# Dave-he/unet-watermark

Hardware: AMD Instinct MI355X
Metric: train_images_per_sec (higher is better)
Workload: dtype f32 storage and accumulation; the convolution products of the encoder and decoder layers (3x3, 7x7 stem, stride-2 and 1x1 layers: forward, data gradients, and the weight gradients of the stride-1 3x3 layers and the stem) as fp16x3 splits - every fp32 operand = two fp16 halves (22 mantissa bits), a*b; 1 GPU; Unet-resnet34 512x512 bs16/GPU train step: fwd + Dice + bwd + Adam (BASELINE.json configs[1]); global_batch=16, parallelism=dp1, grad_allreduce=none

## Files before the change

unet-watermark_amd/_lib.py:

```python
from __future__ import annotations

import ctypes as C
import os
import subprocess
import sys
from pathlib import Path

os.environ.setdefault("GPU_MAX_HW_QUEUES", "8")

_PKG_DIR = Path(__file__).resolve().parent
_CSRC = _PKG_DIR / "csrc"
LIB_PATH = _PKG_DIR / "libuwm.so"
SOURCES = ["uwm_route.hip", "conv_igemm.hip", "conv_patch.hip", "conv_patch16.hip", "conv_wino.hip", "conv_wino8.hip", "conv_wino_x3.hip", "conv_f16x3.hip", "conv_f16x3v2.hip", "conv_stem_f16x3.hip", "conv_up2.hip", "conv_up2_f16.hip", "conv_c16_f16.hip", "conv_gemm.hip", "conv_head.hip", "mbconv.hip", "wgrad_igemm.hip", "wgrad_patch.hip", "wgrad_wino.hip", "wgrad_f16x3.hip", "wgrad_c16.hip", "wgrad_gemm.hip", "wgrad_stem.hip", "elementwise.hip", "loss.hip", "loss_ext.hip", "mask_post.hip", "mask_enhance.hip", "resize_u8.hip", "pair_mask_u8.hip", "synth_u8.hip", "synth_text_u8.hip", "extract_u8.hip", "text_enhance.hip", "filter_u8.hip", "augment_u8.hip", "augment_ext_u8.hip", "jpeg_u8.hip", "uwm_model.hip"]
HIP_ARCH = "gfx950"
EXTRA_FLAGS = {name: ["-Xclang", "-target-feature", "-Xclang", "-packed-fp32-ops"]
               for name in ("conv_f16x3.hip", "conv_f16x3v2.hip", "wgrad_f16x3.hip", "conv_stem_f16x3.hip")}
EXTRA_FLAGS["synth_u8.hip"] = ["-ffp-contract=off"]
EXTRA_FLAGS["synth_text_u8.hip"] = ["-ffp-contract=off"]
EXTRA_FLAGS["extract_u8.hip"] = ["-ffp-contract=off"]
EXTRA_FLAGS["text_enhance.hip"] = ["-ffp-contract=off"]


class uwm_unet_desc(C.Structure):
    _fields_ = [("encoder", C.c_int), ("in_channels", C.c_int), ("classes", C.c_int),
                ("decoder_channels", C.c_int * 5), ("bn_eps", C.c_float), ("bn_momentum", C.c_float), ("arch", C.c_int)]


class uwm_tensor_info(C.Structure):
    _fields_ = [("name", C.c_char * 96), ("kind", C.c_int), ("arena", C.c_int), ("ndim", C.c_int),
                ("offset", C.c_longlong), ("shape", C.c_longlong * 4), ("stride", C.c_longlong * 4)]


class uwm_src(C.Structure):
    _fields_ = [("ptr", C.c_void_p), ("scale", C.c_void_p), ("shift", C.c_void_p),
                ("C", C.c_int), ("H", C.c_int), ("W", C.c_int), ("up", C.c_int), ("relu", C.c_int)]

# ... 252 lines not shown
```

unet-watermark_amd/csrc/elementwise.hip:

```cpp
#include "uwm_kernels.h"
#include <vector>
#include <mutex>
#include <cstdlib>

namespace uwm {

typedef float f4 __attribute__((ext_vector_type(4)));
static constexpr int kMaxBlocks = 256 * 8;

static inline unsigned nblocks(size_t work, int per_block) {
  size_t b = (work + per_block - 1) / per_block;
  if (b > (size_t)kMaxBlocks) b = kMaxBlocks;
  if (b < 1) b = 1;
  return (unsigned)b;
}

__global__ void nchw_to_nhwc4_kernel(const float* __restrict__ x, float* __restrict__ y, int C, size_t HW,
                                     size_t total, int CP) {
  for (size_t i = blockIdx.x * (size_t)blockDim.x + threadIdx.x; i < total; i += (size_t)gridDim.x * blockDim.x) {
    const size_t n = i / HW, p = i - n * HW;
    const float* xp = x + n * C * HW + p;
    float* yp = y + i * CP;
    for (int c0 = 0; c0 < CP; c0 += 4) {
      f4 v;
// ... 800 lines not shown
}
const char* prof_class_name(int cls) {
  static const char* names[kProfClasses] = {
      "conv_igemm_kernel<128,128,2,2>", "conv_igemm_kernel<128,64,2,2>", "conv_igemm_kernel<128,32,4,1>",
      "conv_igemm_kernel<128,16,4,1>",  "conv_igemm_kernel<64,64,2,2>",  "conv_igemm_kernel<64,128,1,4>",
      "wgrad_igemm_kernel<64,128,2,2>", "wgrad_igemm_kernel<128,128,2,2>", "wgrad_igemm_kernel<16,256,1,4>",
      "wgrad_igemm_kernel<32,256,1,4>", "conv_patch_kernel<128,2,2>", "conv_patch_kernel<64,2,2>",
      "conv_patch_kernel<32,4,1>",      "conv_patch_kernel<16,4,1>",      "wgrad_patch_kernel<16>",
      "wgrad_patch_kernel<32>",         "wgrad_patch_kernel<64>",         "conv_patch16_kernel<16>",
      "conv_patch16_kernel<32>",        "conv_wino_kernel<64>",           "conv_wino_kernel<32>",
      "conv_wino_kernel<16>",           "wgrad_wino2_kernel<64>",         "wgrad_wino2_kernel<32>",
      "wgrad_wino_kernel<16>",          "conv_wino8_kernel",              "wgrad_igemm_kernel<128,32,2,2>",
      "wgrad_igemm_kernel<128,64,2,2>",  "wgrad_igemm_kernel<32,64,2,2>",  "wgrad_igemm_kernel<32,128,1,4>",
      "conv_head_kernel",               "conv_wino_x3_kernel",            "wgrad_c16_kernel",
      "wgrad_head_kernel",              "conv_up2_kernel",                "conv_up2_dgrad_kernel",
      "wgrad_up2_kernel",               "conv_gemm_kernel<128>",          "conv_gemm_kernel<64>",
      "wgrad_gemm_kernel<128>",         "wgrad_gemm_kernel<64>",          "wgrad_stem_kernel",
      "conv_f16x3_kernel",              "wgrad_f16x3_kernel",             "conv_stem_f16x3_kernel",
      "conv_up2_f16x3_kernel",          "conv_up2_dgrad_f16x3_kernel",    "wgrad_up2_f16x3_kernel",
      "conv_c16_f16x3_kernel",          "wgrad_c16_f16x3_kernel",         "wgrad_stem_f16x3_kernel",
      "conv_gemm_f16x3_kernel<128>",    "conv_gemm_f16x3_kernel<64>",
      "conv_igemm_f16x3_kernel<128,128,2,2>", "conv_igemm_f16x3_kernel<128,64,2,2>", "conv_igemm_f16x3_kernel<128,32,4,1>",
      "conv_igemm_f16x3_kernel<128,16,4,1>",  "conv_igemm_f16x3_kernel<64,64,2,2>",  "conv_igemm_f16x3_kernel<64,128,1,4>",
      "?", "wgrad_igemm_f16x3_kernel<128,128,2,2>", "wgrad_igemm_f16x3_kernel<128,64,2,2>", "wgrad_igemm_f16x3_kernel<64,128,2,2>", "?"};
  return (cls >= 0 && cls < kProfClasses) ? names[cls] : "?";
}

}
```

unet-watermark_amd/csrc/uwm_abi.inc:

```
extern "C" {

const char* uwm_last_error(void) { return g_err; }
int uwm_version(void) { return 1; }

int uwm_create(const uwm_unet_desc* desc, uwm_handle* out) {
  if (!desc || !out) return fail("uwm_create: null argument");
  uwm_model* m = new uwm_model();
  m->desc = *desc;
  if (m->desc.bn_eps <= 0.f) m->desc.bn_eps = 1e-5f;
  if (m->desc.bn_momentum <= 0.f) m->desc.bn_momentum = 0.1f;
  if (build_model(m)) { delete m; return 1; }
  const char* e = getenv("UWM_SIDE_STREAM");
  m->use_side = e ? atoi(e) : 1;
  if (const char* pe = getenv("UWM_PRECISION")) {
    static const char* names[7] = {"f32", "bf16x3", "bf16x3_all", "f16x3", "f16x3_all", "f16x1", "f16x3_bwd2"};
    int found = -1;
    for (int i = 0; i < 7; ++i) if (!strcmp(pe, names[i]) || (pe[0] == '0' + i && !pe[1])) found = i;
    if (found < 0) { delete m; return fail("uwm_create: UWM_PRECISION=%s is not a precision mode (f32 | bf16x3 | bf16x3_all | f16x3 | f16x3_all | f16x1 | f16x3_bwd2 or 0..6)", pe); }
    m->prec = found; m->plan.prec = found; m->prec_from_env = found != UWM_PREC_F32;
  }
  if (const char* pf = getenv("UWM_F16X3_MIN_WGS")) m->f3_min_wgs = atoi(pf) > 0 ? atoi(pf) : 0;
  m->wino_mode = winograd_mode();
  m->plan.wino_mode = m->wino_mode;
  *out = m; return 0;
// ... 1091 lines not shown
    if (rc != 0) return fail("uwm_allreduce_grads: ncclAllReduce failed on bucket %d (ncclResult_t %d)", k, rc);
  }
  return 0;
}
float* uwm_grad_arena(uwm_handle h) { return h ? h->grads : nullptr; }
static Src to_src(const uwm_src* s) { return mk_src(s->ptr, s->C, s->H, s->W, s->scale, s->shift, s->relu, s->up); }

static int g_op_ig16 = 0;
static int op_ig_bank(const float* w, int rows, int Kpad, int slot, hipStream_t st, const float** bank) {
  static float* buf[2] = {nullptr, nullptr}; static size_t cap[2] = {0, 0};
  const size_t n = (size_t)rows * Kpad;
  if (n > cap[slot]) {
    if (buf[slot]) HIPCHK(hipFree(buf[slot]));
    buf[slot] = nullptr; cap[slot] = 0;
    HIPCHK(hipMalloc((void**)&buf[slot], n * sizeof(float)));
    cap[slot] = n;
  }
  WinoJobs jobs; memset(&jobs, 0, sizeof(jobs)); jobs.n = 1;
  jobs.j[0].w = w; jobs.j[0].ut = buf[slot]; jobs.j[0].rows = rows; jobs.j[0].Kpad = Kpad; jobs.j[0].mode = 3; jobs.j[0].src_rows = rows;
  LCHK(launch_f16x3_weights_multi(jobs, st));
  *bank = buf[slot];
  return 0;
}
int uwm_op_set_igemm_f16x3(int on) { g_op_ig16 = on == 2 ? 2 : (on != 0); return 0; }
int uwm_op_conv(const uwm_src* s0, const uwm_src* s1, const float* w, int wrows, int Kpad, int kh, int kw, int stride,
                int pad, int N, int Cout, const float* bias, float* y, double* stats, int cfg, uwm_stream stream) {
  if (!s0 || !w || !y) return fail("uwm_op_conv: null argument");
  ConvArgs a; memset(&a, 0, sizeof(a));
  a.s0 = to_src(s0); a.C0 = a.s0.C;
  if (s1) { a.s1 = to_src(s1); a.Ctot = a.C0 + a.s1.C; } else { a.s1 = a.s0; a.Ctot = a.C0; }
  a.Hl = a.s0.H << a.s0.up; a.Wl = a.s0.W << a.s0.up;
  a.w = w; a.wrows = wrows; a.Kpad = Kpad; a.ntaps = kh * kw; a.kw = kw;
  a.N = N; a.Ho = (a.Hl + 2 * pad - kh) / stride + 1; a.Wo = (a.Wl + 2 * pad - kw) / stride + 1;
  a.Cout = Cout; a.M = N * a.Ho * a.Wo;
  a.smul = stride; a.rmul = 1; a.off = -pad; a.sdiv = 1;
  a.out = y; a.bias = bias;
  if (stats) { a.ssum = stats; a.ssq = stats + Cout; }
  a.dv_ctot = make_fastdiv(a.Ctot); a.dv_kw = make_fastdiv(a.kw);
  a.ig16 = g_op_ig16 != 0;
  if (g_op_ig16 == 1 && !(Kpad & 31) && cfg < 6 && conv_route(a, cfg).k == kConvIgemm && op_ig_bank(w, wrows, Kpad, 0, (hipStream_t)stream, &a.wbank)) return 1;
  if (cfg == 610) {
    static float* sbuf = nullptr;
    if (!sbuf) HIPCHK(hipMalloc((void**)&sbuf, stem_f16x3_bank_floats() * sizeof(float)));
    if (kh != 7 || kw != 7 || a.Ctot != 4 || wrows != 64) return fail("uwm_op_conv: cfg 610 is the 7x7 stem (4 stored input channels, 64 outputs)");
    LCHK(launch_stem_f16x3_weights(w, Kpad, a.Ctot, sbuf, (hipStream_t)stream));
    a.wu = sbuf;
    LCHK(launch_conv_stem_f16x3(a, (hipStream_t)stream));
// ... 10 lines not shown
  } else if (cfg >= 300 && cfg < 500) return fail("uwm_op_conv: cfg 300 (Winograd) needs 3x3 s1 p1, channels %% 8 == 0, Ho >= 8, Wo >= 16");
  LCHK(launch_conv(a, (hipStream_t)stream, cfg));
  return 0;
}
int uwm_op_dgrad(const float* dy, int N, int Ho, int Wo, int Cout, const float* wd, int Cin, int KpadD, int kh, int kw,
                 int stride, int pad, int H, int W, const float* addend, const float* mask, const float* mscale,
                 const float* mshift, float* dx, uwm_stream stream) {
  if (!dy || !wd || !dx) return fail("uwm_op_dgrad: null argument");
  ConvArgs a; memset(&a, 0, sizeof(a));
  a.s0 = mk_src(dy, Cout, Ho, Wo); a.s1 = a.s0; a.C0 = Cout; a.Ctot = Cout;
  a.w = wd; a.wrows = Cin; a.Kpad = KpadD; a.ntaps = kh * kw; a.kw = kw;
  a.N = N; a.Ho = H; a.Wo = W; a.Cout = Cin; a.M = N * H * W;
  a.Hl = Ho; a.Wl = Wo; a.smul = 1; a.rmul = -1; a.off = pad; a.sdiv = stride;
  a.out = dx; a.addend = addend; a.mask = mask; a.mscale = mscale; a.mshift = mshift;
  a.dv_ctot = make_fastdiv(a.Ctot); a.dv_kw = make_fastdiv(a.kw);
  if (g_op_ig16) {
    static float* xm = nullptr;
    if (!xm) HIPCHK(hipMalloc((void**)&xm, 32 * sizeof(float)));
    LCHK(launch_absmax32(dy, (size_t)N * Ho * Wo * Cout, xm, (hipStream_t)stream));
    a.ig16 = 1; a.xmax = xm;
  }
  if (winograd_mode() != 0 && op_wino_shape(a, kh, kw, stride, pad) && op_wino_prepare(a, 1, (hipStream_t)stream)) return 1;
  if (g_op_ig16 == 1 && !(KpadD & 31)) {
    const ConvKernel k = conv_route(a, -1).k;
    if ((k == kConvIgemm || k == kConvS2Dgrad) && op_ig_bank(wd, Cin, KpadD, 0, (hipStream_t)stream, &a.wbank)) return 1;
  }
  LCHK(launch_conv(a, (hipStream_t)stream));
  return 0;
}
int uwm_op_dgrad_upsplit(const float* dy, int N, int H, int W, int Cout, const float* wd, int C0, int C1, int KpadD,
                         float* gprev, const float* pmask, const float* pscale, const float* pshift, float* gskip,
                         uwm_stream stream) {
  if (!dy || !wd || !gprev || (C1 > 0 && !gskip)) return fail("uwm_op_dgrad_upsplit: null argument");
  ConvArgs a; memset(&a, 0, sizeof(a));
  a.s0 = mk_src(dy, Cout, H, W); a.s1 = a.s0; a.C0 = Cout; a.Ctot = Cout;
  a.w = wd; a.wrows = C0 + C1; a.Kpad = KpadD; a.ntaps = 9; a.kw = 3;
  a.N = N; a.Ho = H; a.Wo = W; a.Cout = C0 + C1; a.M = N * H * W;
  a.Hl = H; a.Wl = W; a.smul = 1; a.rmul = -1; a.off = 1; a.sdiv = 1;
  a.out = gskip; a.out_up = gprev; a.up_c0 = C0; a.up_mask = pmask; a.up_mscale = pscale; a.up_mshift = pshift;
  a.dv_ctot = make_fastdiv(a.Ctot); a.dv_kw = make_fastdiv(a.kw);
  if (!op_wino_shape(a, 3, 3, 1, 1) || (H & 1) || (W & 1)) return fail("uwm_op_dgrad_upsplit: needs even H >= 8, W >= 16, channels %% 8 == 0");
  if (g_op_ig16) {
    static float* xm = nullptr;
    if (!xm) HIPCHK(hipMalloc((void**)&xm, 32 * sizeof(float)));
    LCHK(launch_absmax32(dy, (size_t)N * H * W * Cout, xm, (hipStream_t)stream));
    a.ig16 = 1; a.xmax = xm;
  }
  if (op_wino_prepare(a, 1, (hipStream_t)stream)) return 1;
  LCHK(launch_conv(a, (hipStream_t)stream));
  return 0;
// ... 130 lines not shown
```

unet-watermark_amd/csrc/uwm_kernels.h:

```cpp
#pragma once
#include <hip/hip_runtime.h>
#include <hip/hip_ext.h>
#include <stdint.h>
#include <stddef.h>
#include <atomic>

struct uwm_loss_spec;

namespace uwm {

struct Src {
  const float* ptr;
  const float* scale;
  const float* shift;
  int C, H, W;
  int up;
  int relu;
};

struct FastDiv {
  unsigned mg, d;
};
static inline FastDiv make_fastdiv(unsigned d) {
  FastDiv f; f.d = d; f.mg = (d <= 1) ? 0u : (unsigned)((0x100000000ull / d) + 1ull); return f;
// ... 29 lines not shown
  const float* mscale; const float* mshift;
  double* ssum; double* ssq;
  int srep, sstride;
  const float* bnb_mean; const float* bnb_rstd;
  const float* bnb_y;
  FastDiv dv_ctot, dv_kw;
  double flops;
  double bytes;
  float* out_up; int up_c0; const float* up_mask; const float* up_mscale; const float* up_mshift;
  int up_accum;
  int pc_ntaps[4]; unsigned pc_taps[4];
  int live_ch;
  const float* wu;
  int wu_ncb;
  int wino;
  int prec;
  int wu_rinv_off;
  const float* xmax;
  int route_n;
  int ig16;
  int nprod;
  const float* wbank;
  int wu_layout;
};

template <class A> static inline int route_N(const A& a) { return a.route_n > 0 ? a.route_n : a.N; }
template <class A> static inline long route_M(const A& a) { return a.N > 0 ? (long)a.M / a.N * route_N(a) : (long)a.M; }

#if defined(__HIPCC__)
typedef unsigned uwm_u2 __attribute__((ext_vector_type(2)));
__device__ __forceinline__ void uwm_split4(float x0, float x1, float x2, float x3, uwm_u2& hi, uwm_u2& lo) {
  typedef _Float16 h2_ __attribute__((ext_vector_type(2)));
  const h2_ a = {(_Float16)x0, (_Float16)x1}, b = {(_Float16)x2, (_Float16)x3};
  hi.x = __builtin_bit_cast(unsigned, a); hi.y = __builtin_bit_cast(unsigned, b);
  unsigned l0, l1;
  asm("v_fma_mixlo_f16 %0, %1, -1.0, %2 op_sel_hi:[1,0,0]\n\t"
      "v_fma_mixhi_f16 %0, %1, -1.0, %3 op_sel:[1,0,0] op_sel_hi:[1,0,0]"
      : "=&v"(l0) : "v"(hi.x), "v"(x0), "v"(x1));
  asm("v_fma_mixlo_f16 %0, %1, -1.0, %2 op_sel_hi:[1,0,0]\n\t"
      "v_fma_mixhi_f16 %0, %1, -1.0, %3 op_sel:[1,0,0] op_sel_hi:[1,0,0]"
      : "=&v"(l1) : "v"(hi.y), "v"(x2), "v"(x3));
  lo.x = l0; lo.y = l1;
}
constexpr float kIgWScale = 4096.f;
__device__ __forceinline__ void ig_bank_unit(const float* __restrict__ src, float* __restrict__ dst, size_t i, int Kpad) {
  typedef float f4_ __attribute__((ext_vector_type(4)));
// ... 40 lines not shown
  int nprod;
};

enum { kProfClasses = 64 };
void prof_enable(bool on);
bool prof_on();
void prof_pair(int cls, double flops, double bytes, hipEvent_t* e0, hipEvent_t* e1);
void route_note(const char* kernel);
const char* route_last();
#define UWM_LAUNCH(cls, flops, bytes, kernel, grid, block, lds, st, ...)                                     \
  do {                                                                                                       \
    route_note(#kernel);                                                                                     \
    if (prof_on()) {                                                                                         \
      hipEvent_t e0_, e1_; prof_pair((cls), (flops), (bytes), &e0_, &e1_);                                   \
      hipExtLaunchKernelGGL(kernel, grid, block, lds, st, e0_, e1_, 0, __VA_ARGS__);                         \
    } else {                                                                                                 \
      hipLaunchKernelGGL(kernel, grid, block, lds, st, __VA_ARGS__);                                         \
    }                                                                                                        \
  } while (0)
int  prof_collect(double* out );
const char* prof_class_name(int cls);

enum ConvKernel { kConvInvalid = 0, kConvUp2, kConvUp2F16, kConvUp2Dgrad, kConvUp2DgradF16, kConvC16F16, kConvC32F16, kConvGemm, kConvHead,
                  kConvHeadDgrad, kConvF16x3, kConvF16x3v2, kConvWinoX3, kConvWino, kConvWino8, kConvPatch16, kConvPatch, kConvS2Dgrad, kConvIgemm };
struct ConvRoute { ConvKernel k; int v; };
ConvRoute conv_route(const ConvArgs& a, int force_cfg);
hipError_t launch_conv(const ConvArgs& a, hipStream_t st, int force_cfg = -1);
bool conv_epilogue_carries_bnb(const ConvArgs& a);
enum WgradKernel { kWgradInvalid = 0, kWgradGemm, kWgradUp2, kWgradF16x3, kWgradStem, kWgradC16, kWgradWino, kWgradPatch, kWgradIgemm };
struct WgradRoute { WgradKernel k; int v; };
WgradRoute wgrad_route(const WgradArgs& a);
hipError_t launch_wgrad(const WgradArgs& a, hipStream_t st);
hipError_t launch_conv_igemm(const ConvArgs& a, hipStream_t st, int cfg);
bool conv_s2_dgrad_applicable(const ConvArgs& a);
hipError_t launch_conv_s2_dgrad(const ConvArgs& a, hipStream_t st, int cfg);
hipError_t launch_wgrad_igemm(const WgradArgs& a, hipStream_t st, bool f16);
bool wgrad_patch_applicable(const WgradArgs& a);
hipError_t launch_wgrad_patch(const WgradArgs& a, hipStream_t st);
bool wgrad_wino_applicable(const WgradArgs& a);
hipError_t launch_wgrad_wino(const WgradArgs& a, hipStream_t st);
size_t wgrad_wino_scratch_floats();
float* wgrad_op_scratch();
bool wgrad_c16_applicable(const WgradArgs& a);
hipError_t launch_wgrad_c16(const WgradArgs& a, hipStream_t st);
hipError_t launch_wgrad_reduce(const float* part, int nsplit, size_t n4, float* dw, hipStream_t st, ReduceQueue* rq = nullptr);
hipError_t launch_wgrad_reduce_multi(ReduceQueue& q, hipStream_t st);
bool wgrad_f16x3_applicable(const WgradArgs& a);
hipError_t launch_wgrad_f16x3(const WgradArgs& a, hipStream_t st);
bool wgrad_stem_applicable(const WgradArgs& a);
hipError_t launch_wgrad_stem(const WgradArgs& a, hipStream_t st);
bool wgrad_gemm_applicable(const WgradArgs& a);
hipError_t launch_wgrad_gemm(const WgradArgs& a, hipStream_t st);
bool wgrad_gemm_preferred(const WgradArgs& a);
bool wgrad_up2_applicable(const WgradArgs& a);
hipError_t launch_wgrad_up2(const WgradArgs& a, hipStream_t st);
bool conv_gemm_applicable(const ConvArgs& a);
hipError_t launch_conv_gemm(const ConvArgs& a, hipStream_t st, int bn);
bool conv_gemm_preferred(const ConvArgs& a);
// ... 328 lines not shown
```

unet-watermark_amd/csrc/uwm_launch.inc:

```
struct Ctx {
  uwm_model* m; float* ws; hipStream_t st; int N;
  hipStream_t wst = nullptr;
  float* fz = nullptr;
  float* F(size_t off) const { return ws + off; }
  const float* bn_ss(const BNL& b) const { return fz ? fz + b.fz_off : ws + b.f_off + 2 * b.C; }
  float* wu(const ConvL& cv) const { return fz ? fz + cv.fz_wu : ws + cv.wu_off; }
  double* D(size_t doff) const { return (double*)ws + doff; }
};
static Src mk_src(const float* ptr, int C, int H, int W, const float* scale = nullptr, const float* shift = nullptr,
                  int relu = 0, int up = 0) {
  Src s; s.ptr = ptr; s.scale = scale; s.shift = shift; s.C = C; s.H = H; s.W = W; s.up = up; s.relu = relu; return s;
}
static Src lazy_src(const Ctx& c, int conv, int H, int W, int relu = 1, int up = 0) {
  const ConvL& cv = c.m->convs[conv];
  const BNL& b = c.m->bns[cv.bn];
  return mk_src(c.F(c.m->plan.y[conv]), cv.CoutP, H, W, c.bn_ss(b), c.bn_ss(b) + b.C, relu, up);
}

static thread_local bool g_err_own = false;
static hipError_t fail_launch(const char* fmt, ...) {
  va_list ap; va_start(ap, fmt); vsnprintf(g_err, sizeof(g_err), fmt, ap); va_end(ap);
  g_err_own = true;
  return hipErrorInvalidValue;
}
// ... 66 lines not shown
  a.N = c.N; a.Ho = Hin; a.Wo = Win; a.Cout = cv.CinP; a.M = c.N * Hin * Win;
  a.Hl = Ho; a.Wl = Wo; a.smul = 1; a.rmul = -1; a.off = cv.pad; a.sdiv = cv.stride;
  a.out = dx; a.addend = addend; a.mask = mask; a.mscale = mscale; a.mshift = mshift; a.live_ch = cv.Cout;
  a.dv_ctot = make_fastdiv(a.Ctot); a.dv_kw = make_fastdiv(a.kw);
  a.flops = 2.0 * (double)c.N * Ho * Wo * cv.Cout * cv.Cin * cv.k * cv.k;
  a.bytes = 4.0 * ((double)c.N * Ho * Wo * cv.CoutP + (double)cv.CinP * cv.KpadD +
                   (double)a.M * cv.CinP * (1.0 + (addend ? 1.0 : 0.0) + (mask ? 1.0 : 0.0)));
  if (cv.wud_off && c.m->plan.wino_ok((size_t)ci)) {
    a.wu = c.F(cv.wud_off); a.wu_ncb = wino_ncb(cv.CinP);
    const int pm = c.m->plan.prec;
    if ((pm == UWM_PREC_BF16X3 || pm == UWM_PREC_BF16X3_ALL) && cv.x3_d()) a.prec = 1;
    if (f3_dgrad_on(c.m, (size_t)ci)) {
      a.prec = 2; a.wu_layout = f3_layout(c.m, (size_t)ci, true); a.nprod = f3_nprod(c.m, true);
      a.wu_ncb = a.wu_layout == 1 ? f16x3v2_nf(cv.CinP) : f16x3_nj(cv.CinP); a.wu_rinv_off = (int)f16x3_rinv_off(cv.CinP, cv.CoutP);
    }
  }
  a.wino = c.m->plan.wino_mode + 1;
  if (conv_ig16(c.m, (size_t)ci, true)) a.ig16 = 1;
  if (ig_bank_on(c.m, (size_t)ci, true)) a.wbank = c.F(cv.wdb_off);
  if (a.prec == 2 || a.ig16) {
    const hipError_t e = dy_max_slot(c, ci, "dgrad", &a.xmax);
    if (e != hipSuccess) return e;
  }
  if (us) { a.out_up = us->gprev; a.up_c0 = us->C0; a.up_mask = us->pmask; a.up_mscale = us->pscale; a.up_mshift = us->pshift; a.up_accum = us->accumulate; }
  if (fused) *fused = false;
  static const bool no_fuse = dbg_flag("UWM_NO_BN_FUSE");
  a.bnb_y = bn_y;
  if (bn_fuse >= 0 && fused && !no_fuse && (us ? (us->pmask != nullptr && !us->accumulate) : (mask != nullptr || bn_y != nullptr)) && conv_epilogue_carries_bnb(a)) {
    const BNL& b = c.m->bns[bn_fuse];
    if (b.C == (us ? us->C0 : cv.CinP)) {
      const float* f = c.F(b.f_off);
      a.bnb_mean = f; a.bnb_rstd = f + b.C;
      a.ssum = c.D(b.d_off) + 2 * b.C; a.ssq = a.ssum + b.C; a.srep = b.nrep; a.sstride = 2 * b.C;
      *fused = true;
    }
  }
  if (!fused || !*fused) a.bnb_y = nullptr;
  a.route_n = c.m->route_n;
  return route_rec(c, "dgrad", ci, launch_conv(a, c.st));
}

static hipError_t run_wgrad(const Ctx& c, int ci, const Src& s0, const Src* s1, const float* dy, int Ho, int Wo) {
  const ConvL& cv = c.m->convs[ci];
  WgradArgs a; memset(&a, 0, sizeof(a));
  a.s0 = s0; a.C0 = s0.C;
  if (s1) { a.s1 = *s1; a.Ctot = s0.C + s1->C; } else { a.s1 = s0; a.Ctot = s0.C; }
// ... 122 lines not shown
```

unet-watermark_amd/csrc/uwm_route.hip:

```cpp
#include "uwm_kernels.h"
#include <stdio.h>
#include <stdlib.h>

namespace uwm {

static int g_winograd = -1;
bool winograd_enabled() {
  if (g_winograd < 0) { const char* e = getenv("UWM_WINOGRAD"); g_winograd = (e && e[0] == '0') ? 0 : 1; }
  return g_winograd != 0;
}
void winograd_set_mode(int mode) { g_winograd = mode; }
int winograd_mode() { (void)winograd_enabled(); return g_winograd; }
int device_cu_count() {
  static int cus[64] = {0};
  int dev = 0; (void)hipGetDevice(&dev);
  if (dev < 0 || dev >= 64) return 256;
  if (!cus[dev] && (hipDeviceGetAttribute(&cus[dev], hipDeviceAttributeMultiprocessorCount, dev) != hipSuccess || cus[dev] <= 0)) cus[dev] = 256;
  return cus[dev];
}

struct RouteSwitches {
  bool trace = dbg_flag("UWM_TRACE_CONV");
  bool no_up2 = dbg_flag("UWM_NO_UP2"), no_up2_wgrad = dbg_flag("UWM_NO_UP2_WGRAD"), no_head = dbg_flag("UWM_NO_CONV_HEAD");
  bool no_bnb_y = dbg_flag("UWM_NO_BNB_Y"), no_igemm_bnb = dbg_flag("UWM_NO_IGEMM_BNB");
  bool no_narrow_1x1 = dbg_flag("UWM_NO_NARROW_1X1"), no_wgrad_ig16 = dbg_flag("UWM_NO_WGRAD_IG16");
};
static const RouteSwitches& switches() { static const RouteSwitches s; return s; }

struct ConvCaps { bool bnb, bnb_y, out_up, bnb_out_up; };
static ConvCaps conv_caps(ConvKernel k) {
  switch (k) {
    case kConvWino:         return {true, true, true, true};
    case kConvWinoX3:       return {true, false, true, true};
    case kConvF16x3:        return {true, true, true, false};
    case kConvUp2Dgrad: case kConvUp2DgradF16: return {true, false, true, true};
    case kConvF16x3v2: case kConvGemm: case kConvS2Dgrad: case kConvIgemm: return {true, true, false, false};
    case kConvC16F16: case kConvC32F16: case kConvPatch16: case kConvHeadDgrad: return {true, false, false, false};
    default:                return {false, false, false, false};
  }
}
ConvRoute conv_route(const ConvArgs& a, int cfg) {
  const RouteSwitches& sw = switches();
  const bool aut = cfg < 0;
  const ConvRoute invalid = {kConvInvalid, 0};
  auto wino = [&](int bn) -> ConvRoute {
    if (bn == 8 || (bn <= 0 && !a.bnb_mean && !a.bnb_y && !a.out_up && conv_wino8_applicable(a))) return {kConvWino8, 0};
    return {kConvWino, bn};
  };
  auto up2 = [&]() -> ConvRoute { return {a.ig16 ? kConvUp2F16 : kConvUp2, 0}; };
  if (cfg == 700) return up2();
  if (cfg == 710 || (aut && a.ig16 && a.prec != 2 && conv_c16_f16_applicable(a))) return {kConvC16F16, 0};
  if (cfg == 711 || (aut && a.ig16 && a.prec != 2 && conv_c32_f16_applicable(a))) return {kConvC32F16, 0};
  if (cfg >= 800 && cfg < 1000) return {kConvGemm, cfg - 800};
  if (cfg == 500) return {kConvHead, 0};
  if ((cfg >= 600 && cfg <= 607) || (aut && a.prec == 2)) {
    const int v = aut ? 0 : cfg - 600;
    if (a.wu_layout == 1) return (v == 4 || v == 6 || !conv_f16x3v2_applicable(a)) ? invalid : ConvRoute{kConvF16x3v2, v == 5};
    return (v >= 4 || !conv_f16x3_applicable(a)) ? invalid : ConvRoute{kConvF16x3, v};
  }
  if (cfg == 400) return {kConvWinoX3, 0};
  if (cfg >= 300) return cfg < 400 ? wino(cfg - 300) : invalid;
  if (a.out_up) {
    if (aut && !sw.no_up2 && conv_up2_dgrad_applicable(a)) return {a.ig16 ? kConvUp2DgradF16 : kConvUp2Dgrad, 0};
    if (a.prec == 1) return conv_wino_x3_applicable(a) ? ConvRoute{kConvWinoX3, 0} : invalid;
    return conv_wino_applicable(a) ? wino(0) : invalid;
  }
  if (cfg == 200) return {kConvPatch16, 0};
  if (aut && !sw.no_up2 && conv_up2_applicable(a)) return up2();
  if (aut && !sw.no_head && conv_head_applicable(a)) return {kConvHead, 0};
  if (aut && !sw.no_head && conv_head_dgrad_applicable(a)) return {kConvHeadDgrad, 0};
  if (aut && wino_mode_of(a.wino) != 0 && conv_wino_applicable(a) && !conv_patch16_applicable(a))
    return a.prec == 1 ? ConvRoute{kConvWinoX3, 0} : wino(0);
  if (cfg >= 100) return {kConvPatch, cfg - 100};
  if (aut && conv_patch16_applicable(a)) return {kConvPatch16, 0};
  if (aut && conv_patch_applicable(a)) {
    const long sp = (long)route_N(a) * ((a.Ho + 7) / 8) * ((a.Wo + 15) / 16);
    int bn = a.Cout >= 128 ? 128 : (a.Cout > 32 ? 64 : (a.Cout > 16 ? 32 : 16));
    if (bn == 128 && sp * ((a.Cout + 127) / 128) < 512) bn = 64;
    return {kConvPatch, bn};
  }
  if (aut && conv_s2_dgrad_applicable(a)) {
    const long t128 = (long)((route_N(a) * (a.Ho >> 1) * (a.Wo >> 1) + 127) / 128) * ((a.Cout + 127) / 128);
    if (a.Cout > 64 && t128 < device_cu_count()) return {kConvS2Dgrad, 4};
    return {kConvS2Dgrad, a.Cout <= 64 ? 1 : 0};
  }
  if (aut && conv_gemm_preferred(a)) return {kConvGemm, 0};
  if (aut) {
    const long tiles128 = (long)((route_M(a) + 127) / 128);
    if (a.Cout <= 16) cfg = 3;
    else if (a.Cout <= 32) cfg = 2;
    else if (a.Cout <= 64) cfg = (tiles128 >= 512) ? 1 : 4;
    else {
      const long b0 = tiles128 * ((a.Cout + 127) / 128);
      const int pad128 = ((a.Cout + 127) / 128) * 128, pad64 = ((a.Cout + 63) / 64) * 64;
      if (!sw.no_narrow_1x1 && a.ntaps == 1 && pad128 * 100 > pad64 * 115 && tiles128 * (pad64 / 64) >= 512) cfg = 1;
      else if (b0 >= 512) cfg = 0;
      else if (tiles128 * ((a.Cout + 63) / 64) >= 512) cfg = 1;
      else cfg = 4;
    }
  }
  return cfg <= 5 ? ConvRoute{kConvIgemm, cfg} : invalid;
}

bool conv_epilogue_carries_bnb(const ConvArgs& a) {
  const ConvKernel k = conv_route(a, -1).k;
  const ConvCaps c = conv_caps(k);
  if (a.out_up) return c.bnb_out_up && !a.bnb_y;
  if (a.bnb_y) return c.bnb_y && a.prec != 1 && !switches().no_bnb_y;
  if (switches().no_igemm_bnb && (k == kConvGemm || k == kConvS2Dgrad || k == kConvIgemm)) return false;
  return c.bnb;
}

hipError_t launch_conv(const ConvArgs& a, hipStream_t st, int force_cfg) {
  if (a.M <= 0 || a.Cout <= 0 || (a.Cout & 3) || (a.Kpad & 31) || (a.Ctot & 3) || (a.C0 & 3)) return hipErrorInvalidValue;
  if (switches().trace)
    fprintf(stderr, "conv %s N=%d Ctot=%d(C0=%d up=%d) Cout=%d Ho=%d Wo=%d Hl=%d Wl=%d taps=%d smul=%d sdiv=%d wino=%d gflop=%.2f\n",
            a.rmul < 0 ? "dgrad" : "fwd", a.N, a.Ctot, a.C0, a.s0.up, a.Cout, a.Ho, a.Wo, a.Hl, a.Wl, a.ntaps, a.smul, a.sdiv,
            (int)(force_cfg < 0 && wino_mode_of(a.wino) != 0 && conv_wino_applicable(a)), a.flops * 1e-9);
  const ConvRoute r = conv_route(a, force_cfg);
  const ConvCaps c = conv_caps(r.k);
  if (a.bnb_mean && (!c.bnb || (a.bnb_y && !c.bnb_y) || (a.out_up && !c.bnb_out_up) || !a.ssum || !a.ssq || !a.bnb_rstd ||
                     !(a.out_up ? a.up_mask : (a.bnb_y ? a.bnb_y : a.mask)) || a.up_accum))
    return hipErrorInvalidValue;
  if (a.out_up && (!c.out_up || ((a.Ho | a.Wo) & 1) || (a.up_c0 & 3) || a.up_c0 > a.Cout || a.addend || a.mask || a.bias || a.bnb_y ||
                   (a.ssum && !a.bnb_mean) || (a.up_c0 < a.Cout && !a.out)))
    return hipErrorInvalidValue;
  switch (r.k) {
    case kConvUp2:         return launch_conv_up2(a, st);
    case kConvUp2F16:      return launch_conv_up2_f16(a, st);
    case kConvUp2Dgrad:    return launch_conv_up2_dgrad(a, st);
    case kConvUp2DgradF16: return launch_conv_up2_dgrad_f16(a, st);
    case kConvC16F16:      return launch_conv_c16_f16(a, st);
    case kConvC32F16:      return launch_conv_c32_f16(a, st);
    case kConvGemm:        return launch_conv_gemm(a, st, r.v);
    case kConvHead:        return launch_conv_head(a, st);
    case kConvHeadDgrad:   return launch_conv_head_dgrad(a, st);
    case kConvF16x3:       return launch_conv_f16x3(a, st, r.v);
    case kConvF16x3v2:     return launch_conv_f16x3v2(a, st, r.v != 0);
    case kConvWinoX3:      return launch_conv_wino_x3(a, st);
    case kConvWino:        return launch_conv_wino(a, st, r.v);
    case kConvWino8:       return launch_conv_wino8(a, st);
    case kConvPatch16:     return launch_conv_patch16(a, st);
    case kConvPatch:       return launch_conv_patch(a, st, r.v);
    case kConvS2Dgrad:     return launch_conv_s2_dgrad(a, st, r.v);
    case kConvIgemm:       return launch_conv_igemm(a, st, r.v);
    default:               return hipErrorInvalidValue;
  }
}

WgradRoute wgrad_route(const WgradArgs& a) {
  const RouteSwitches& sw = switches();
  const int f = a.force_igemm & 0xff;
  const bool aut = f == 0, no_up2 = sw.no_up2 || sw.no_up2_wgrad;
  if (f == 4) return {kWgradGemm, 0};
  if (a.prec == 2 && (aut || f == 6)) {
    if (a.xmax && !no_up2 && wgrad_up2_applicable(a) && wgrad_up2_f16_shape(a)) return {kWgradUp2, 0};
    if (wgrad_f16x3_applicable(a)) return {kWgradF16x3, 0};
  }
  if (f == 6) {
    if (a.prec == 2 && wgrad_stem_applicable(a)) return {kWgradStem, 0};
    if (a.prec == 2 && a.Cout == 16 && wgrad_c16_applicable(a)) return {kWgradC16, 0};
    return {kWgradInvalid, 0};
  }
  if (aut && !no_up2 && wgrad_up2_applicable(a)) return {kWgradUp2, 0};
  if (aut && wgrad_stem_applicable(a)) return {kWgradStem, 0};
  if (aut && wgrad_gemm_preferred(a)) return {kWgradGemm, 0};
// ... 28 lines not shown
```

Before: 1233 images/s.

## Add direct fp16x3 MFMA kernel for stride-2 3x3 data-gradient convolutions

```diff
diff --git a/unet-watermark_amd/_lib.py b/unet-watermark_amd/_lib.py
--- a/unet-watermark_amd/_lib.py
+++ b/unet-watermark_amd/_lib.py
@@ -11,7 +11,7 @@
 _PKG_DIR = Path(__file__).resolve().parent
 _CSRC = _PKG_DIR / "csrc"
 LIB_PATH = _PKG_DIR / "libuwm.so"
-SOURCES = ["uwm_route.hip", "conv_igemm.hip", "conv_patch.hip", "conv_patch16.hip", "conv_wino.hip", "conv_wino8.hip", "conv_wino_x3.hip", "conv_f16x3.hip", "conv_f16x3v2.hip", "conv_stem_f16x3.hip", "conv_up2.hip", "conv_up2_f16.hip", "conv_c16_f16.hip", "conv_gemm.hip", "conv_head.hip", "mbconv.hip", "wgrad_igemm.hip", "wgrad_patch.hip", "wgrad_wino.hip", "wgrad_f16x3.hip", "wgrad_c16.hip", "wgrad_gemm.hip", "wgrad_stem.hip", "elementwise.hip", "loss.hip", "loss_ext.hip", "mask_post.hip", "mask_enhance.hip", "resize_u8.hip", "pair_mask_u8.hip", "synth_u8.hip", "synth_text_u8.hip", "extract_u8.hip", "text_enhance.hip", "filter_u8.hip", "augment_u8.hip", "augment_ext_u8.hip", "jpeg_u8.hip", "uwm_model.hip"]
+SOURCES = ["uwm_route.hip", "conv_igemm.hip", "conv_patch.hip", "conv_patch16.hip", "conv_wino.hip", "conv_wino8.hip", "conv_wino_x3.hip", "conv_f16x3.hip", "conv_f16x3v2.hip", "conv_f16x3_s2.hip", "conv_stem_f16x3.hip", "conv_up2.hip", "conv_up2_f16.hip", "conv_c16_f16.hip", "conv_gemm.hip", "conv_head.hip", "mbconv.hip", "wgrad_igemm.hip", "wgrad_patch.hip", "wgrad_wino.hip", "wgrad_f16x3.hip", "wgrad_c16.hip", "wgrad_gemm.hip", "wgrad_stem.hip", "elementwise.hip", "loss.hip", "loss_ext.hip", "mask_post.hip", "mask_enhance.hip", "resize_u8.hip", "pair_mask_u8.hip", "synth_u8.hip", "synth_text_u8.hip", "extract_u8.hip", "text_enhance.hip", "filter_u8.hip", "augment_u8.hip", "augment_ext_u8.hip", "jpeg_u8.hip", "uwm_model.hip"]
 HIP_ARCH = "gfx950"
 EXTRA_FLAGS = {name: ["-Xclang", "-target-feature", "-Xclang", "-packed-fp32-ops"]
                for name in ("conv_f16x3.hip", "conv_f16x3v2.hip", "wgrad_f16x3.hip", "conv_stem_f16x3.hip")}
diff --git a/unet-watermark_amd/csrc/conv_f16x3_s2.hip b/unet-watermark_amd/csrc/conv_f16x3_s2.hip
--- /dev/null
+++ b/unet-watermark_amd/csrc/conv_f16x3_s2.hip
@@ -0,0 +1,258 @@
+#include "uwm_kernels.h"
+
+namespace uwm {
+
+typedef float f4 __attribute__((ext_vector_type(4)));
+typedef _Float16 h8 __attribute__((ext_vector_type(8)));
+typedef unsigned u4 __attribute__((ext_vector_type(4)));
+
+constexpr int kS2W = 16;
+constexpr int kS2H = 8;
+constexpr int kS2Pix = 72;
+constexpr int kS2QLd = 36;
+constexpr int kS2Co = 32;
+
+__device__ __forceinline__ float s2_clamp_h(float v) { return __builtin_amdgcn_fmed3f(v, -65504.f, 65504.f); }
+
+constexpr size_t kS2Lds = (size_t)(kS2H + 1) * (kS2W + 1) * kS2Pix * sizeof(_Float16) + (size_t)9 * kS2Co * 128;
+
+template <bool WB>
+__global__ __launch_bounds__(256, 2) void conv_f16x3_s2_dgrad_kernel(const ConvArgs a) {
+  constexpr int TH = kS2H;
+  constexpr int RW = TH / 4;
+  constexpr int PW = kS2W + 1, PH = TH + 1, NPX = PH * PW;
+  constexpr int NU = NPX * 8;
+  constexpr int NR = (NU + 255) / 256;
+  extern __shared__ __attribute__((aligned(16))) _Float16 hsm[];
+
+  const int tid = threadIdx.x, lane = tid & 63, wave = __builtin_amdgcn_readfirstlane(tid >> 6);
+  const int px16 = lane & 15, g = lane >> 4;
+
+  const unsigned nblk = gridDim.x, bid = blockIdx.x;
+  const unsigned q8 = nblk >> 3, r8 = nblk & 7, xcd = bid & 7;
+  unsigned tile = (xcd < r8 ? xcd * (q8 + 1) : r8 * (q8 + 1) + (xcd - r8) * q8) + (bid >> 3);
+  const int tilesN = a.Cout / kS2Co;
+  const int tilesW = (a.Wl + kS2W - 1) / kS2W, tilesH = (a.Hl + TH - 1) / TH;
+  const int tn = tile % tilesN; tile /= tilesN;
+  const int tw = tile % tilesW; tile /= tilesW;
+  const int th = tile % tilesH; const int n = tile / tilesH;
+  const int n0 = tn * kS2Co, i0 = th * TH, j0 = tw * kS2W;
+  const int nchunk = a.Ctot >> 5;
+
+  float xs = 1.f;
+  if (a.xmax) {
+    float mx = a.xmax[lane & 31];
+#pragma unroll
+    for (int d = 16; d >= 1; d >>= 1) mx = fmaxf(mx, __shfl_xor(mx, d));
+    if (mx > 0.f && mx < 3.0e38f) { int e; (void)frexpf(mx, &e); xs = ldexpf(1.f, 14 - e); }
+  }
+
+  f4 acc[RW][4][2];
+#pragma unroll
+  for (int i = 0; i < RW; ++i)
+#pragma unroll
+    for (int c = 0; c < 4; ++c)
+#pragma unroll
+      for (int j = 0; j < 2; ++j) acc[i][c][j] = (f4){0.f, 0.f, 0.f, 0.f};
+
+  int goff[NR];
+  unsigned gflags = 0;
+#pragma unroll
+  for (int rd = 0; rd < NR; ++rd) {
+    const int u = rd * 256 + tid;
+    const bool act = u < NU;
+    const int pp = act ? (u >> 3) : 0;
+    const int pr = pp / PW, pcx = pp - pr * PW;
+    const int hl = i0 + pr, wl = j0 + pcx;
+    const bool ok = act && hl < a.Hl && wl < a.Wl;
+    const int hc = min(hl, a.Hl - 1), wc = min(wl, a.Wl - 1);
+    goff[rd] = ((n * a.Hl + hc) * a.Wl + wc) * a.Ctot + (u & 7) * 4;
+    gflags |= ((ok ? 1u : 0u) | (act ? 0x10000u : 0u)) << rd;
+  }
+  f4 pv[NR];
+  auto patch_load = [&](int c) {
+    const float* sp = a.s0.ptr + c * 32;
+#pragma unroll
+    for (int rd = 0; rd < NR; ++rd) pv[rd] = *(const f4*)(sp + goff[rd]);
+  };
+  auto patch_store = [&]() {
+#pragma unroll
+    for (int rd = 0; rd < NR; ++rd) {
+      f4 v = pv[rd] * xs;
+      if (!((gflags >> rd) & 1u)) v = (f4){0.f, 0.f, 0.f, 0.f};
+      uwm_u2 hi, lo;
+      uwm_split4(s2_clamp_h(v.x), s2_clamp_h(v.y), s2_clamp_h(v.z), s2_clamp_h(v.w), hi, lo);
+      if ((gflags >> (16 + rd)) & 1u) {
+        const int u = rd * 256 + tid;
+        _Float16* d = hsm + (u >> 3) * kS2Pix + (u & 7) * 4;
+        *(uwm_u2*)d = hi;
+        *(uwm_u2*)(d + 32) = lo;
+      }
+    }
+  };
+
+  char* const wl = (char*)(hsm + NPX * kS2Pix);
+  const int wu_row = tid >> 3, wu_unit = tid & 7;
+  const float* const wsrc = (WB ? a.wbank : a.w) + (size_t)(n0 + wu_row) * a.Kpad + wu_unit * 4;
+  f4 wv[9];
+  auto w_gload = [&](int c) {
+#pragma unroll
+    for (int t = 0; t < 9; ++t) wv[t] = *(const f4*)(wsrc + t * a.Ctot + c * 32);
+  };
+  auto w_lstore = [&]() {
+    const int sw = (wu_row >> 1) & 7;
+#pragma unroll
+    for (int t = 0; t < 9; ++t) {
+      char* rb = wl + (t * 32 + wu_row) * 128;
+      if (WB) *(f4*)(rb + wu_unit * 16) = wv[t];
+      else {
+        const f4 w4 = wv[t] * kIgWScale;
+        uwm_u2 hi, lo;
+        uwm_split4(s2_clamp_h(w4.x), s2_clamp_h(w4.y), s2_clamp_h(w4.z), s2_clamp_h(w4.w), hi, lo);
+        *(uwm_u2*)(rb + (((wu_unit >> 1) ^ sw) << 4) + (wu_unit & 1) * 8) = hi;
+        *(uwm_u2*)(rb + ((((wu_unit >> 1) + 4) ^ sw) << 4) + (wu_unit & 1) * 8) = lo;
+      }
+    }
+  };
+  const int asw = (px16 >> 1) & 7;
+  const char* const abase = wl + px16 * 128;
+  const int aoff_hi = (g ^ asw) << 4, aoff_lo = ((g + 4) ^ asw) << 4;
+  const int pbase = ((wave * RW) * PW + px16) * kS2Pix + g * 8;
+  h8 xh[RW + 1][2], xl[RW + 1][2];
+  auto x_read = [&]() {
+#pragma unroll
+    for (int i = 0; i <= RW; ++i)
+#pragma unroll
+      for (int d = 0; d < 2; ++d) {
+        const _Float16* pp = hsm + pbase + (i * PW + d) * kS2Pix;
+        xh[i][d] = *(const h8*)pp; xl[i][d] = *(const h8*)(pp + 32);
+      }
+  };
+  auto mma_tap = [&](int t) {
+    const int r = t / 3, s = t - r * 3;
+    const int cls = (r != 1 ? 2 : 0) + (s != 1 ? 1 : 0), dyo = r == 0 ? 1 : 0, dxo = s == 0 ? 1 : 0;
+    h8 whi[2], wlo[2];
+#pragma unroll
+    for (int j = 0; j < 2; ++j) {
+      const char* p = abase + (t * 32 + j * 16) * 128;
+      whi[j] = *(const h8*)(p + aoff_hi); wlo[j] = *(const h8*)(p + aoff_lo);
+    }
+#pragma unroll
+    for (int i = 0; i < RW; ++i)
+#pragma unroll
+      for (int j = 0; j < 2; ++j) acc[i][cls][j] = __builtin_amdgcn_mfma_f32_16x16x32_f16(whi[j], xh[i + dyo][dxo], acc[i][cls][j], 0, 0, 0);
+#pragma unroll
+    for (int i = 0; i < RW; ++i)
+#pragma unroll
+      for (int j = 0; j < 2; ++j) acc[i][cls][j] = __builtin_amdgcn_mfma_f32_16x16x32_f16(whi[j], xl[i + dyo][dxo], acc[i][cls][j], 0, 0, 0);
+#pragma unroll
+    for (int i = 0; i < RW; ++i)
+#pragma unroll
+      for (int j = 0; j < 2; ++j) acc[i][cls][j] = __builtin_amdgcn_mfma_f32_16x16x32_f16(wlo[j], xh[i + dyo][dxo], acc[i][cls][j], 0, 0, 0);
+  };
+
+  patch_load(0); w_gload(0);
+  patch_store(); w_lstore();
+  if (nchunk > 1) { patch_load(1); w_gload(1); }
+  __syncthreads();
+  for (int c = 0; c < nchunk; ++c) {
+    x_read();
+#pragma unroll
+    for (int t = 0; t < 9; ++t) mma_tap(t);
+    __syncthreads();
+    if (c + 1 < nchunk) {
+      patch_store(); w_lstore();
+      if (c + 2 < nchunk) { patch_load(c + 2); w_gload(c + 2); }
+    }
+    __syncthreads();
+  }
+
+  float* const R = (float*)hsm + wave * 32 * kS2QLd;
+  const float unscale = 1.f / (kIgWScale * xs);
+  const bool do_stats = a.ssum != nullptr;
+  const bool bnb = a.bnb_mean != nullptr;
+  const int cq = lane & 7, sub = lane >> 3;
+  const int co = n0 + cq * 4;
+  f4 ps_ = {0.f, 0.f, 0.f, 0.f}, pq_ = ps_;
+  f4 bmu = ps_, brs = ps_, bia = ps_, msc = {1.f, 1.f, 1.f, 1.f}, msh = ps_;
+  if (bnb) { bmu = *(const f4*)(a.bnb_mean + co); brs = *(const f4*)(a.bnb_rstd + co); }
+  if (a.bias) bia = *(const f4*)(a.bias + co);
+  if (a.mscale) { msc = *(const f4*)(a.mscale + co); msh = *(const f4*)(a.mshift + co); }
+#pragma unroll
+  for (int i = 0; i < RW; ++i) {
+#pragma unroll
+    for (int py = 0; py < 2; ++py) {
+#pragma unroll
+      for (int px = 0; px < 2; ++px)
+#pragma unroll
+        for (int j = 0; j < 2; ++j) *(f4*)(R + (2 * px16 + px) * kS2QLd + j * 16 + g * 4) = acc[i][py * 2 + px][j];
+      __syncthreads();
+      const int ho = 2 * (i0 + wave * RW + i) + py;
+#pragma unroll
+      for (int r = 0; r < 4; ++r) {
+        const int p = r * 8 + sub;
+        const int wo = 2 * j0 + p;
+        if (ho < a.Ho && wo < a.Wo) {
+          const size_t o = (((size_t)n * a.Ho + ho) * a.Wo + wo) * a.Cout + co;
+          f4 v = *(const f4*)(R + p * kS2QLd + cq * 4) * unscale + bia;
+          if (a.addend) v += *(const f4*)(a.addend + o);
+          f4 yr = {0.f, 0.f, 0.f, 0.f};
+          if (a.mask) {
+            f4 mk = *(const f4*)(a.mask + o);
+            yr = mk;
+            if (a.mscale) mk = mk * msc + msh;
+            v.x = mk.x > 0.f ? v.x : 0.f; v.y = mk.y > 0.f ? v.y : 0.f;
+            v.z = mk.z > 0.f ? v.z : 0.f; v.w = mk.w > 0.f ? v.w : 0.f;
+          }
+          *(f4*)(a.out + o) = v;
+          if (a.bnb_y) yr = *(const f4*)(a.bnb_y + o);
+          ps_ += v; pq_ += bnb ? v * ((yr - bmu) * brs) : v * v;
+        }
+      }
+      __syncthreads();
+    }
+  }
+  if (do_stats) {
+#pragma unroll
+    for (int e = 0; e < 4; ++e) {
+      float sv = ps_[e], qv = pq_[e];
+#pragma unroll
+      for (int d = 8; d < 64; d <<= 1) { sv += __shfl_xor(sv, d); qv += __shfl_xor(qv, d); }
+      ps_[e] = sv; pq_[e] = qv;
+    }
+    float* red = (float*)hsm;
+    if (sub == 0) {
+#pragma unroll
+      for (int e = 0; e < 4; ++e) { red[(wave * kS2Co + cq * 4 + e) * 2] = ps_[e]; red[(wave * kS2Co + cq * 4 + e) * 2 + 1] = pq_[e]; }
+    }
+    __syncthreads();
+    if (tid < kS2Co) {
+      double sv = 0.0, qv = 0.0;
+#pragma unroll
+      for (int w = 0; w < 4; ++w) { sv += (double)red[(w * kS2Co + tid) * 2]; qv += (double)red[(w * kS2Co + tid) * 2 + 1]; }
+      const size_t srep_off = a.srep > 1 ? (size_t)(blockIdx.x & (unsigned)(a.srep - 1)) * a.sstride : 0;
+      atomicAdd(a.ssum + srep_off + n0 + tid, sv);
+      atomicAdd(a.ssq + srep_off + n0 + tid, qv);
+    }
+  }
+}
+
+bool conv_f16x3_s2_dgrad_applicable(const ConvArgs& a) {
+  return a.ig16 && a.rmul == -1 && a.sdiv == 2 && a.smul == 1 && a.off == 1 && a.ntaps == 9 && a.kw == 3 && (a.Ctot & 31) == 0 &&
+         a.C0 == a.Ctot && (a.Cout & 31) == 0 && a.wrows == a.Cout && a.Kpad >= 9 * a.Ctot && a.Ho == 2 * a.Hl && a.Wo == 2 * a.Wl &&
+         a.s0.up == 0 && a.s0.scale == nullptr && !a.s0.relu && a.s0.H == a.Hl && a.s0.W == a.Wl && a.s0.C == a.Ctot && !a.out_up &&
+         a.out != nullptr && (double)a.N * a.Hl * a.Wl * a.Ctot < 2.0e9 && (a.wbank != nullptr || a.w != nullptr);
+}
+long conv_f16x3_s2_dgrad_wgs(const ConvArgs& a, int n) {
+  return (long)n * ((a.Hl + kS2H - 1) / kS2H) * ((a.Wl + kS2W - 1) / kS2W) * (a.Cout / kS2Co);
+}
+hipError_t launch_conv_f16x3_s2_dgrad(const ConvArgs& a, hipStream_t st) {
+  if (!conv_f16x3_s2_dgrad_applicable(a)) return hipErrorInvalidValue;
+  const unsigned grid = (unsigned)conv_f16x3_s2_dgrad_wgs(a, a.N);
+  if (a.wbank) UWM_LAUNCH(59, a.flops, a.bytes, (conv_f16x3_s2_dgrad_kernel<true>), dim3(grid), dim3(256), kS2Lds, st, a);
+  else UWM_LAUNCH(59, a.flops, a.bytes, (conv_f16x3_s2_dgrad_kernel<false>), dim3(grid), dim3(256), kS2Lds, st, a);
+  route_note("(conv_f16x3_s2_dgrad_kernel)");
+  return hipGetLastError();
+}
+
+}
diff --git a/unet-watermark_amd/csrc/elementwise.hip b/unet-watermark_amd/csrc/elementwise.hip
--- a/unet-watermark_amd/csrc/elementwise.hip
+++ b/unet-watermark_amd/csrc/elementwise.hip
@@ -846,7 +846,7 @@
       "conv_gemm_f16x3_kernel<128>",    "conv_gemm_f16x3_kernel<64>",
       "conv_igemm_f16x3_kernel<128,128,2,2>", "conv_igemm_f16x3_kernel<128,64,2,2>", "conv_igemm_f16x3_kernel<128,32,4,1>",
       "conv_igemm_f16x3_kernel<128,16,4,1>",  "conv_igemm_f16x3_kernel<64,64,2,2>",  "conv_igemm_f16x3_kernel<64,128,1,4>",
-      "?", "wgrad_igemm_f16x3_kernel<128,128,2,2>", "wgrad_igemm_f16x3_kernel<128,64,2,2>", "wgrad_igemm_f16x3_kernel<64,128,2,2>", "?"};
+      "conv_f16x3_s2_dgrad_kernel", "wgrad_igemm_f16x3_kernel<128,128,2,2>", "wgrad_igemm_f16x3_kernel<128,64,2,2>", "wgrad_igemm_f16x3_kernel<64,128,2,2>", "?"};
   return (cls >= 0 && cls < kProfClasses) ? names[cls] : "?";
 }
 
diff --git a/unet-watermark_amd/csrc/uwm_abi.inc b/unet-watermark_amd/csrc/uwm_abi.inc
--- a/unet-watermark_amd/csrc/uwm_abi.inc
+++ b/unet-watermark_amd/csrc/uwm_abi.inc
@@ -1137,7 +1137,14 @@
   *bank = buf[slot];
   return 0;
 }
-int uwm_op_set_igemm_f16x3(int on) { g_op_ig16 = on == 2 ? 2 : (on != 0); return 0; }
+static int g_op_dgrad_cfg = -1;
+int uwm_op_set_igemm_f16x3(int on) {
+  static const int codes[3] = {-1, 620, 625};
+  const int s2 = on >> 4;
+  if (on < 0 || s2 > 2) return fail("uwm_op_set_igemm_f16x3: bad mode %d", on);
+  on &= 15;
+  g_op_ig16 = on == 2 ? 2 : (on != 0); g_op_dgrad_cfg = codes[s2]; return 0;
+}
 int uwm_op_conv(const uwm_src* s0, const uwm_src* s1, const float* w, int wrows, int Kpad, int kh, int kw, int stride,
                 int pad, int N, int Cout, const float* bias, float* y, double* stats, int cfg, uwm_stream stream) {
   if (!s0 || !w || !y) return fail("uwm_op_conv: null argument");
@@ -1194,10 +1201,12 @@
   }
   if (winograd_mode() != 0 && op_wino_shape(a, kh, kw, stride, pad) && op_wino_prepare(a, 1, (hipStream_t)stream)) return 1;
   if (g_op_ig16 == 1 && !(KpadD & 31)) {
-    const ConvKernel k = conv_route(a, -1).k;
-    if ((k == kConvIgemm || k == kConvS2Dgrad) && op_ig_bank(wd, Cin, KpadD, 0, (hipStream_t)stream, &a.wbank)) return 1;
-  }
-  LCHK(launch_conv(a, (hipStream_t)stream));
+    const ConvKernel k = conv_route(a, g_op_dgrad_cfg).k;
+    if ((k == kConvIgemm || k == kConvS2Dgrad || k == kConvF16x3S2Dgrad) && op_ig_bank(wd, Cin, KpadD, 0, (hipStream_t)stream, &a.wbank)) return 1;
+  }
+  if (g_op_dgrad_cfg == 620 && !conv_f16x3_s2_dgrad_applicable(a))
+    return fail("uwm_op_dgrad: code %d (conv_f16x3_s2.hip) needs uwm_op_set_igemm_f16x3 mode 1 | 2, 3x3 s2 p1, channels %% 32 == 0, H == 2 Ho, W == 2 Wo", g_op_dgrad_cfg);
+  LCHK(launch_conv(a, (hipStream_t)stream, g_op_dgrad_cfg));
   return 0;
 }
 int uwm_op_dgrad_upsplit(const float* dy, int N, int H, int W, int Cout, const float* wd, int C0, int C1, int KpadD,
diff --git a/unet-watermark_amd/csrc/uwm_kernels.h b/unet-watermark_amd/csrc/uwm_kernels.h
--- a/unet-watermark_amd/csrc/uwm_kernels.h
+++ b/unet-watermark_amd/csrc/uwm_kernels.h
@@ -75,6 +75,7 @@
   int nprod;
   const float* wbank;
   int wu_layout;
+  int min_wgs;
 };
 
 template <class A> static inline int route_N(const A& a) { return a.route_n > 0 ? a.route_n : a.N; }
@@ -161,7 +162,7 @@
 const char* prof_class_name(int cls);
 
 enum ConvKernel { kConvInvalid = 0, kConvUp2, kConvUp2F16, kConvUp2Dgrad, kConvUp2DgradF16, kConvC16F16, kConvC32F16, kConvGemm, kConvHead,
-                  kConvHeadDgrad, kConvF16x3, kConvF16x3v2, kConvWinoX3, kConvWino, kConvWino8, kConvPatch16, kConvPatch, kConvS2Dgrad, kConvIgemm };
+                  kConvHeadDgrad, kConvF16x3, kConvF16x3v2, kConvWinoX3, kConvWino, kConvWino8, kConvPatch16, kConvPatch, kConvF16x3S2Dgrad, kConvS2Dgrad, kConvIgemm };
 struct ConvRoute { ConvKernel k; int v; };
 ConvRoute conv_route(const ConvArgs& a, int force_cfg);
 hipError_t launch_conv(const ConvArgs& a, hipStream_t st, int force_cfg = -1);
@@ -173,6 +174,9 @@
 hipError_t launch_conv_igemm(const ConvArgs& a, hipStream_t st, int cfg);
 bool conv_s2_dgrad_applicable(const ConvArgs& a);
 hipError_t launch_conv_s2_dgrad(const ConvArgs& a, hipStream_t st, int cfg);
+bool conv_f16x3_s2_dgrad_applicable(const ConvArgs& a);
+long conv_f16x3_s2_dgrad_wgs(const ConvArgs& a, int n);
+hipError_t launch_conv_f16x3_s2_dgrad(const ConvArgs& a, hipStream_t st);
 hipError_t launch_wgrad_igemm(const WgradArgs& a, hipStream_t st, bool f16);
 bool wgrad_patch_applicable(const WgradArgs& a);
 hipError_t launch_wgrad_patch(const WgradArgs& a, hipStream_t st);
diff --git a/unet-watermark_amd/csrc/uwm_launch.inc b/unet-watermark_amd/csrc/uwm_launch.inc
--- a/unet-watermark_amd/csrc/uwm_launch.inc
+++ b/unet-watermark_amd/csrc/uwm_launch.inc
@@ -112,6 +112,7 @@
     const hipError_t e = dy_max_slot(c, ci, "dgrad", &a.xmax);
     if (e != hipSuccess) return e;
   }
+  a.min_wgs = c.m->f3_min_wgs;
   if (us) { a.out_up = us->gprev; a.up_c0 = us->C0; a.up_mask = us->pmask; a.up_mscale = us->pscale; a.up_mshift = us->pshift; a.up_accum = us->accumulate; }
   if (fused) *fused = false;
   static const bool no_fuse = dbg_flag("UWM_NO_BN_FUSE");
diff --git a/unet-watermark_amd/csrc/uwm_route.hip b/unet-watermark_amd/csrc/uwm_route.hip
--- a/unet-watermark_amd/csrc/uwm_route.hip
+++ b/unet-watermark_amd/csrc/uwm_route.hip
@@ -24,6 +24,7 @@
   bool no_up2 = dbg_flag("UWM_NO_UP2"), no_up2_wgrad = dbg_flag("UWM_NO_UP2_WGRAD"), no_head = dbg_flag("UWM_NO_CONV_HEAD");
   bool no_bnb_y = dbg_flag("UWM_NO_BNB_Y"), no_igemm_bnb = dbg_flag("UWM_NO_IGEMM_BNB");
   bool no_narrow_1x1 = dbg_flag("UWM_NO_NARROW_1X1"), no_wgrad_ig16 = dbg_flag("UWM_NO_WGRAD_IG16");
+  bool no_s2_direct = dbg_flag("UWM_NO_S2_DIRECT");
 };
 static const RouteSwitches& switches() { static const RouteSwitches s; return s; }
 
@@ -34,13 +35,15 @@
     case kConvWinoX3:       return {true, false, true, true};
     case kConvF16x3:        return {true, true, true, false};
     case kConvUp2Dgrad: case kConvUp2DgradF16: return {true, false, true, true};
-    case kConvF16x3v2: case kConvGemm: case kConvS2Dgrad: case kConvIgemm: return {true, true, false, false};
+    case kConvF16x3v2: case kConvGemm: case kConvF16x3S2Dgrad: case kConvS2Dgrad: case kConvIgemm: return {true, true, false, false};
     case kConvC16F16: case kConvC32F16: case kConvPatch16: case kConvHeadDgrad: return {true, false, false, false};
     default:                return {false, false, false, false};
   }
 }
 ConvRoute conv_route(const ConvArgs& a, int cfg) {
   const RouteSwitches& sw = switches();
+  const bool no_s2_direct = sw.no_s2_direct || cfg == 625;
+  if (cfg == 625) cfg = -1;
   const bool aut = cfg < 0;
   const ConvRoute invalid = {kConvInvalid, 0};
   auto wino = [&](int bn) -> ConvRoute {
@@ -48,6 +51,7 @@
     return {kConvWino, bn};
   };
   auto up2 = [&]() -> ConvRoute { return {a.ig16 ? kConvUp2F16 : kConvUp2, 0}; };
+  if (cfg == 620) return conv_f16x3_s2_dgrad_applicable(a) ? ConvRoute{kConvF16x3S2Dgrad, 0} : invalid;
   if (cfg == 700) return up2();
   if (cfg == 710 || (aut && a.ig16 && a.prec != 2 && conv_c16_f16_applicable(a))) return {kConvC16F16, 0};
   if (cfg == 711 || (aut && a.ig16 && a.prec != 2 && conv_c32_f16_applicable(a))) return {kConvC32F16, 0};
@@ -79,6 +83,9 @@
     if (bn == 128 && sp * ((a.Cout + 127) / 128) < 512) bn = 64;
     return {kConvPatch, bn};
   }
+  if (aut && !no_s2_direct && conv_f16x3_s2_dgrad_applicable(a) &&
+      conv_f16x3_s2_dgrad_wgs(a, route_N(a)) >= (a.min_wgs > 0 ? a.min_wgs : device_cu_count() / 2))
+    return {kConvF16x3S2Dgrad, 0};
   if (aut && conv_s2_dgrad_applicable(a)) {
     const long t128 = (long)((route_N(a) * (a.Ho >> 1) * (a.Wo >> 1) + 127) / 128) * ((a.Cout + 127) / 128);
     if (a.Cout > 64 && t128 < device_cu_count()) return {kConvS2Dgrad, 4};
@@ -107,7 +114,7 @@
   const ConvCaps c = conv_caps(k);
   if (a.out_up) return c.bnb_out_up && !a.bnb_y;
   if (a.bnb_y) return c.bnb_y && a.prec != 1 && !switches().no_bnb_y;
-  if (switches().no_igemm_bnb && (k == kConvGemm || k == kConvS2Dgrad || k == kConvIgemm)) return false;
+  if (switches().no_igemm_bnb && (k == kConvGemm || k == kConvF16x3S2Dgrad || k == kConvS2Dgrad || k == kConvIgemm)) return false;
   return c.bnb;
 }
 
@@ -142,6 +149,7 @@
     case kConvWino8:       return launch_conv_wino8(a, st);
     case kConvPatch16:     return launch_conv_patch16(a, st);
     case kConvPatch:       return launch_conv_patch(a, st, r.v);
+    case kConvF16x3S2Dgrad: return launch_conv_f16x3_s2_dgrad(a, st);
     case kConvS2Dgrad:     return launch_conv_s2_dgrad(a, st, r.v);
     case kConvIgemm:       return launch_conv_igemm(a, st, r.v);
     default:               return hipErrorInvalidValue;
```

Result: no change. 1244 images/s, median of 6 (+0.9%).
